# violetdenim/c3dgs

Measured on AMD Instinct MI355X. Metric: raster views/sec fwd+bwd @1920x1080, higher is better.
Workload: dtype f32; 1 GPU; BASELINE.json configs[2]: synth-v1 3M Gaussians, SH deg 3, indexed-camera rasterizer (QAT inner loop), mark_visible+fwd+bwd, 1 view/step/GPU; gaussians=3000000, width=1920, height=1080, sh_codebook=304096, gaussian_codebook=754096, parallelism=replicas x1

## Files before the change

### c3dgs_amd/csrc/backward_preprocess.hip

```cpp
#include "common.hpp"
#include "gsmath.hpp"

#ifndef C3DGS_BWD_CH
#define C3DGS_BWD_CH 128
#endif
#ifndef C3DGS_BWD_LONG_RUN
#define C3DGS_BWD_LONG_RUN 32
#endif
#ifndef C3DGS_BWD_FG
#define C3DGS_BWD_FG 8
#endif
#ifndef C3DGS_BWD_WAVES
#define C3DGS_BWD_WAVES 3
#endif

namespace c3dgs {

constexpr int SUM_WAVES = BWD_LIST / 64;
static_assert(BWD_LIST % 256 == 0 && BWD_LIST <= 1024, "a list is one workgroup of sum_partials_kernel and whole ones of backward_preprocess_kernel");

struct BwdArgs {
    int P, D, M, W, H;
    const float* means3D; const float* sh; const float* scales; const float* scale_factors; const float* rotations;
    const float* cov3D_precomp; const int64_t* sh_indices; const int64_t* g_indices;
    const float* view; const float* proj; const float* campos;
    float tan_fovx, tan_fovy, focal_x, focal_y, scale_modifier;
    const int32_t* radii; const uint32_t* inst_offset; const uint32_t* block_base; const uint8_t* clamped; const float4* splat;
    float* partials; const uint8_t* touched;
    uint32_t* live_count; uint32_t* live_ids; uint32_t* live_slots;
    c3dgs_raster_grads g;
};

template <int DEG>
__device__ __forceinline__ void sh_backward(const float* c, const f3 d0, const float g[3], float dmean_add[3], float* basis_out)
{
    const float len = sqrtf(d0.x * d0.x + d0.y * d0.y + d0.z * d0.z);
    const float x = d0.x / len, y = d0.y / len, z = d0.z / len;
    float dx[3] = { 0, 0, 0 }, dy[3] = { 0, 0, 0 }, dz[3] = { 0, 0, 0 };
    constexpr int NB = (DEG + 1) * (DEG + 1);
    float basis[NB];
    basis[0] = SH_C0;
    if (DEG > 0) {
        basis[1] = -SH_C1 * y; basis[2] = SH_C1 * z; basis[3] = -SH_C1 * x;
#pragma unroll
        for (int ch = 0; ch < 3; ch++) {
            dx[ch] = -SH_C1 * c[3 * 3 + ch];
            dy[ch] = -SH_C1 * c[1 * 3 + ch];
            dz[ch] = SH_C1 * c[2 * 3 + ch];
        }
    }
    if (DEG > 1) {
        const float xx = x * x, yy = y * y, zz = z * z, xy = x * y, yz = y * z, xz = x * z;
        basis[4] = SH_C2_0 * xy; basis[5] = SH_C2_1 * yz; basis[6] = SH_C2_2 * (2.f * zz - xx - yy);
        basis[7] = SH_C2_3 * xz; basis[8] = SH_C2_4 * (xx - yy);
#pragma unroll
        for (int ch = 0; ch < 3; ch++) {
            const float s4 = c[4 * 3 + ch], s5 = c[5 * 3 + ch], s6 = c[6 * 3 + ch], s7 = c[7 * 3 + ch], s8 = c[8 * 3 + ch];
            dx[ch] += SH_C2_0 * y * s4 + SH_C2_2 * 2.f * -x * s6 + SH_C2_3 * z * s7 + SH_C2_4 * 2.f * x * s8;
            dy[ch] += SH_C2_0 * x * s4 + SH_C2_1 * z * s5 + SH_C2_2 * 2.f * -y * s6 + SH_C2_4 * 2.f * -y * s8;
            dz[ch] += SH_C2_1 * y * s5 + SH_C2_2 * 2.f * 2.f * z * s6 + SH_C2_3 * x * s7;
        }
        if (DEG > 2) {
            basis[9] = SH_C3_0 * y * (3.f * xx - yy);
            basis[10] = SH_C3_1 * xy * z;
            basis[11] = SH_C3_2 * y * (4.f * zz - xx - yy);
            basis[12] = SH_C3_3 * z * (2.f * zz - 3.f * xx - 3.f * yy);
            basis[13] = SH_C3_4 * x * (4.f * zz - xx - yy);
            basis[14] = SH_C3_5 * z * (xx - yy);
            basis[15] = SH_C3_6 * x * (xx - 3.f * yy);
#pragma unroll
            for (int ch = 0; ch < 3; ch++) {
                const float s9 = c[9 * 3 + ch], s10 = c[10 * 3 + ch], s11 = c[11 * 3 + ch], s12 = c[12 * 3 + ch],
                            s13 = c[13 * 3 + ch], s14 = c[14 * 3 + ch], s15 = c[15 * 3 + ch];
                dx[ch] += SH_C3_0 * s9 * 3.f * 2.f * xy + SH_C3_1 * s10 * yz + SH_C3_2 * s11 * -2.f * xy +
                          SH_C3_3 * s12 * -3.f * 2.f * xz + SH_C3_4 * s13 * (-3.f * xx + 4.f * zz - yy) +
                          SH_C3_5 * s14 * 2.f * xz + SH_C3_6 * s15 * 3.f * (xx - yy);
                dy[ch] += SH_C3_0 * s9 * 3.f * (xx - yy) + SH_C3_1 * s10 * xz + SH_C3_2 * s11 * (-3.f * yy + 4.f * zz - xx) +
                          SH_C3_3 * s12 * -3.f * 2.f * yz + SH_C3_4 * s13 * -2.f * xy + SH_C3_5 * s14 * -2.f * yz +
                          SH_C3_6 * s15 * -3.f * 2.f * xy;
                dz[ch] += SH_C3_1 * s10 * xy + SH_C3_2 * s11 * 4.f * 2.f * yz + SH_C3_3 * s12 * 3.f * (2.f * zz - xx - yy) +
                          SH_C3_4 * s13 * 4.f * 2.f * xz + SH_C3_5 * s14 * (xx - yy);
            }
        }
    }
#pragma unroll
    for (int k = 0; k < NB; k++) basis_out[k] = basis[k];
    const float ddx = dx[0] * g[0] + dx[1] * g[1] + dx[2] * g[2];
    const float ddy = dy[0] * g[0] + dy[1] * g[1] + dy[2] * g[2];
    const float ddz = dz[0] * g[0] + dz[1] * g[1] + dz[2] * g[2];
    const float sum2 = d0.x * d0.x + d0.y * d0.y + d0.z * d0.z;
    const float invsum32 = 1.0f / sqrtf(sum2 * sum2 * sum2);
    dmean_add[0] = ((+sum2 - d0.x * d0.x) * ddx - d0.y * d0.x * ddy - d0.z * d0.x * ddz) * invsum32;
    dmean_add[1] = (-d0.x * d0.y * ddx + (sum2 - d0.y * d0.y) * ddy - d0.z * d0.y * ddz) * invsum32;
    dmean_add[2] = (-d0.x * d0.z * ddx - d0.y * d0.z * ddy + (sum2 - d0.z * d0.z) * ddz) * invsum32;
}

__device__ __forceinline__ uint32_t nth_set_bit(unsigned long long m, uint32_t r)
{
    uint32_t w = (uint32_t)m, at = 0, c = (uint32_t)__popc(w);
    if (r >= c) { r -= c; w = (uint32_t)(m >> 32); at = 32; }
    c = (uint32_t)__popc(w & 0xFFFFu); if (r >= c) { r -= c; w >>= 16; at += 16; }
    c = (uint32_t)__popc(w & 0xFFu);   if (r >= c) { r -= c; w >>= 8; at += 8; }
    c = (uint32_t)__popc(w & 0xFu);    if (r >= c) { r -= c; w >>= 4; at += 4; }
    c = (uint32_t)__popc(w & 0x3u);    if (r >= c) { r -= c; w >>= 2; at += 2; }
    if (r >= (w & 1u)) at += 1;
    return at;
}

__global__ void __launch_bounds__(BWD_LIST) __attribute__((amdgpu_waves_per_eu(8, 8))) sum_partials_kernel(const BwdArgs a)
{
    constexpr int SW = SUM_WAVES, LIST = BWD_LIST;
    const int i = blockIdx.x * LIST + threadIdx.x;
    const size_t si = (size_t)i;
    const c3dgs_raster_grads& o = a.g;

    constexpr int CH = C3DGS_BWD_CH;
    __shared__ float s_buf[SUM_WAVES][CH * PARTIAL_FLOATS];
#define s_stage(w, sl, q) s_buf[w][(sl) * PARTIAL_FLOATS + (q)]
    constexpr int FG = C3DGS_BWD_FG;
    __shared__ unsigned long long s_fl[SUM_WAVES][FG];
    __shared__ uint32_t s_pre[SUM_WAVES][FG + 1];
    bool any_written = false;
    float acc[PARTIAL_FLOATS];
#pragma unroll
    for (int q = 0; q < PARTIAL_FLOATS; q++) acc[q] = 0.f;
    const int lane_ = threadIdx.x & 63, wv = threadIdx.x >> 6;
    const unsigned long long lt_mask = (1ull << lane_) - 1ull;
    uint32_t start_;
    {
        const int ic = min(i, a.P - 1);
        const uint32_t end_ = a.inst_offset[ic] + a.block_base[ic >> 8];
        start_ = (ic == 0) ? 0u : a.inst_offset[ic - 1] + a.block_base[(ic - 1) >> 8];
        if (i >= a.P) start_ = end_;
        const uint32_t w_begin = __builtin_amdgcn_readfirstlane(start_);
        const uint32_t w_end = __builtin_amdgcn_readlane(end_, 63);
        for (uint32_t base = w_begin; base < w_end; base += FG * 64) {
            const uint32_t nsl = min((uint32_t)(FG * 64), w_end - base);
            uint32_t fbits = 0;
            uint8_t fb[FG];
#pragma unroll
            for (int g = 0; g < FG; g++) fb[g] = a.touched[base + min((uint32_t)(g * 64 + lane_), nsl - 1u)];
#pragma unroll
            for (int g = 0; g < FG; g++)
                if ((uint32_t)(g * 64 + lane_) < nsl && fb[g] != 0) fbits |= 1u << g;
            uint32_t W = 0;
            uint32_t pre[FG + 1];
#pragma unroll
            for (int g = 0; g < FG; g++) {
                const unsigned long long bm = __ballot((fbits >> g) & 1u);
                if (lane_ == 0) { s_fl[wv][g] = bm; s_pre[wv][g] = W; }
                pre[g] = W;
                W += (uint32_t)__popcll(bm);
            }
            pre[FG] = W;
            if (W == 0) continue;
            if (lane_ == 0) s_pre[wv][FG] = W;
            __builtin_amdgcn_fence(__ATOMIC_RELEASE, "wavefront");
            __builtin_amdgcn_wave_barrier();
            __builtin_amdgcn_fence(__ATOMIC_ACQUIRE, "wavefront");
            auto below = [&](uint32_t x) -> uint32_t {
                const uint32_t g = x >> 6;
                if (g >= (uint32_t)FG) return s_pre[wv][FG];
                return s_pre[wv][g] + (uint32_t)__popcll(s_fl[wv][g] & ((1ull << (x & 63u)) - 1ull));
            };
            const uint32_t lo = min(max(start_, base), base + nsl) - base, hi = min(max(end_, base), base + nsl) - base;
            const uint32_t clo = below(lo), chi = below(hi);
            any_written |= chi > clo;
            for (uint32_t p0 = 0; p0 < W; p0 += CH) {
                float st[CH / 64][PARTIAL_FLOATS];
#pragma unroll
                for (int h = 0; h < CH / 64; h++) {
                    const uint32_t e = min(p0 + (uint32_t)(h * 64 + lane_), W - 1u);
                    uint32_t g = 0, r = e;
#pragma unroll
                    for (int k = 1; k < FG; k++)
                        if (e >= pre[k]) { g = (uint32_t)k; r = e - pre[k]; }
                    const uint32_t slot = g * 64u + nth_set_bit(s_fl[wv][g], r);
                    const float* src = a.partials + (size_t)(base + slot) * PARTIAL_FLOATS;
#pragma unroll
                    for (int q = 0; q < PARTIAL_FLOATS; q++) st[h][q] = src[q];
                }
#pragma unroll
                for (int h = 0; h < CH / 64; h++)
#pragma unroll
                    for (int q = 0; q < PARTIAL_FLOATS; q++) s_stage(wv, h * 64 + lane_, q) = st[h][q];
                __builtin_amdgcn_fence(__ATOMIC_RELEASE, "wavefront");
                __builtin_amdgcn_wave_barrier();
                __builtin_amdgcn_fence(__ATOMIC_ACQUIRE, "wavefront");
                const uint32_t c_lo = max(clo, p0), c_hi = min(chi, p0 + CH);
                const bool long_run = c_hi > c_lo + (uint32_t)C3DGS_BWD_LONG_RUN;
                unsigned long long longm = __ballot(long_run);
                while (longm) {
                    const int owner = __ffsll((long long)longm) - 1;
                    longm &= longm - 1ull;
                    const uint32_t o_lo = (uint32_t)__shfl((int)c_lo, owner) - p0, o_hi = (uint32_t)__shfl((int)c_hi, owner) - p0;
                    float part[PARTIAL_FLOATS];
#pragma unroll
                    for (int q = 0; q < PARTIAL_FLOATS; q++) part[q] = 0.f;
                    for (uint32_t e = o_lo + (uint32_t)lane_; e < o_hi; e += 64u) {
#pragma unroll
                        for (int q = 0; q < PARTIAL_FLOATS; q++) part[q] += s_stage(wv, e, q);
                    }
#pragma unroll
                    for (int q = 0; q < PARTIAL_FLOATS; q++) {
#pragma unroll
                        for (int o = 32; o > 0; o >>= 1) part[q] += __shfl_xor(part[q], o);
                        if (lane_ == owner) acc[q] += part[q];
                    }
                }
                if (!long_run) {
                    for (uint32_t c = c_lo; c < c_hi; c++) {
#pragma unroll
                        for (int q = 0; q < PARTIAL_FLOATS; q++) acc[q] += s_stage(wv, c - p0, q);
                    }
                }
                __builtin_amdgcn_fence(__ATOMIC_RELEASE, "wavefront");
                __builtin_amdgcn_wave_barrier();
            }
        }
    }
    const bool live = any_written;
    const unsigned long long lm = __ballot(live);
    const bool per_gaussian_rows = !a.sh_indices && !a.g_indices;
    bool sh_rows_done = false;
    if (per_gaussian_rows && o.dL_dsh && a.sh && ((a.M * 3) & 3) == 0 && (reinterpret_cast<uintptr_t>(o.dL_dsh) & 15u) == 0) {
        sh_rows_done = true;
        const int r4 = (a.M * 3) >> 2;
        const int first = blockIdx.x * LIST + wv * 64;
        const int rows = min(64, a.P - first);
        float4* span = reinterpret_cast<float4*>(o.dL_dsh + (size_t)first * a.M * 3);
        int row = lane_ / r4, col = lane_ - row * r4;
        const int drow = 64 / r4, dcol = 64 - drow * r4;
        for (int q = lane_; q < rows * r4; q += 64) {
            if (!((lm >> row) & 1ull)) span[q] = make_float4(0.f, 0.f, 0.f, 0.f);
            row += drow; col += dcol;
            if (col >= r4) { col -= r4; row++; }
        }
    }
    if (i < a.P && !live) {
        if (o.dL_dmeans2D) { o.dL_dmeans2D[3 * si] = 0.f; o.dL_dmeans2D[3 * si + 1] = 0.f; o.dL_dmeans2D[3 * si + 2] = 0.f; }
        if (o.dL_dcolors) { o.dL_dcolors[3 * si] = 0.f; o.dL_dcolors[3 * si + 1] = 0.f; o.dL_dcolors[3 * si + 2] = 0.f; }
        if (o.dL_dopacity) o.dL_dopacity[si] = 0.f;
        if (o.dL_dmeans3D) { o.dL_dmeans3D[3 * si] = 0.f; o.dL_dmeans3D[3 * si + 1] = 0.f; o.dL_dmeans3D[3 * si + 2] = 0.f; }
        if (o.dL_dcov3D) for (int q = 0; q < 6; q++) o.dL_dcov3D[6 * si + q] = 0.f;
        if (o.dL_dscale_factors) o.dL_dscale_factors[si] = 0.f;
        if (per_gaussian_rows) {
            if (o.dL_dsh && a.sh && !sh_rows_done) for (int q = 0; q < a.M * 3; q++) o.dL_dsh[si * a.M * 3 + q] = 0.f;
            if (o.dL_dscales && a.scales) for (int q = 0; q < 3; q++) o.dL_dscales[3 * si + q] = 0.f;
            if (o.dL_drotations && a.scales) for (int q = 0; q < 4; q++) o.dL_drotations[4 * si + q] = 0.f;
        }
    }
    __shared__ uint32_t s_cnt[SW];
    if (lane_ == 0) s_cnt[wv] = (uint32_t)__popcll(lm);
    __syncthreads();
    uint32_t run0 = 0, all = 0;
#pragma unroll
    for (int w = 0; w < SW; w++) { const uint32_t c = s_cnt[w]; run0 += (w < wv) ? c : 0u; all += c; }
    if (live) {
        const size_t pos = (size_t)blockIdx.x * LIST + run0 + (uint32_t)__popcll(lm & lt_mask);
        a.live_ids[pos] = (uint32_t)i;
        a.live_slots[pos] = start_;
        float* dst = a.partials + (size_t)start_ * PARTIAL_FLOATS;
#pragma unroll
        for (int q = 0; q < PARTIAL_FLOATS; q++) dst[q] = acc[q];
    }
    if (threadIdx.x == 0) a.live_count[blockIdx.x] = all;
}
#undef s_stage

template <int DEG, bool INDEXED>
__global__ void __launch_bounds__(256)
#if C3DGS_BWD_WAVES
__attribute__((amdgpu_waves_per_eu(C3DGS_BWD_WAVES, C3DGS_BWD_WAVES)))
#endif
backward_preprocess_kernel(const BwdArgs a, const float* __restrict__ cam_view, const float* __restrict__ cam_proj,
                           const float* __restrict__ cam_pos)
{
    const uint32_t n_lists = gridDim.x / (BWD_LIST / 256);
    const uint32_t list = blockIdx.x % n_lists, quarter = blockIdx.x / n_lists;
    const uint32_t n_live = a.live_count[list];
    const uint32_t off = quarter * 256u + threadIdx.x;
    if ((off & ~63u) >= n_live) return;
    const size_t pos = (size_t)list * BWD_LIST + off;
    const bool live = off < n_live;
    const int i = live ? (int)a.live_ids[pos] : 0;
    const size_t si = (size_t)i;
    const c3dgs_raster_grads& o = a.g;
    constexpr int NB = (DEG + 1) * (DEG + 1);

    __shared__ float s_g[256][3];
    __shared__ int32_t s_row[256];
    __shared__ float s_ds[INDEXED ? 256 : 1][3];
    __shared__ float s_dq[INDEXED ? 256 : 1][4];
    __shared__ int32_t s_gi[INDEXED ? 256 : 1];
    __shared__ float s_bas[256][NB + 1];
#define s_basis(t, k) s_bas[t][k]
    s_row[threadIdx.x] = -1;
    if (INDEXED) s_gi[threadIdx.x] = -1;

    if (live) {
    float acc[PARTIAL_FLOATS];
    {
        const float* src = a.partials + (size_t)a.live_slots[pos] * PARTIAL_FLOATS;
#pragma unroll
        for (int q = 0; q < PARTIAL_FLOATS; q++) acc[q] = src[q];
    }
    const float4 rec0 = a.splat[3 * si], rec1 = a.splat[3 * si + 1];
    const f3 m = { a.means3D[3 * si], a.means3D[3 * si + 1], a.means3D[3 * si + 2] };
    const uint8_t cl = a.clamped[i];
    size_t gi = si, row = si;
    float sf = 1.f;
    if (INDEXED) {
        if (a.g_indices) gi = (size_t)a.g_indices[i];
        if (a.scale_factors) sf = a.scale_factors[i];
        if (a.sh_indices) row = (size_t)a.sh_indices[i];
    }
    float sc[3] = { 0, 0, 0 };
    float4 rot = make_float4(1, 0, 0, 0);
    float cov3D[6];
    if (a.cov3D_precomp) {
#pragma unroll
        for (int q = 0; q < 6; q++) cov3D[q] = a.cov3D_precomp[6 * si + q];
    } else {
        sc[0] = a.scales[3 * gi]; sc[1] = a.scales[3 * gi + 1]; sc[2] = a.scales[3 * gi + 2];
        rot = *reinterpret_cast<const float4*>(a.rotations + 4 * gi);
    }
    constexpr int NC = (DEG + 1) * (DEG + 1) * 3;
    float c[NC];
    if (a.sh) {
        const float* shp = a.sh + row * (size_t)a.M * 3;
        if ((a.M * 3) % 4 == 0 && NC % 4 == 0) {
#pragma unroll
            for (int q = 0; q < NC / 4; q++) {
                const float4 v = reinterpret_cast<const float4*>(shp)[q];
                c[4 * q] = v.x; c[4 * q + 1] = v.y; c[4 * q + 2] = v.z; c[4 * q + 3] = v.w;
            }
        } else {
#pragma unroll
            for (int q = 0; q < NC; q++) c[q] = shp[q];
        }
    }

    float sh_add[3] = { 0.f, 0.f, 0.f };
    if (a.sh) {
        const float g[3] = { (cl & 1) ? 0.f : acc[0], (cl & 2) ? 0.f : acc[1], (cl & 4) ? 0.f : acc[2] };
        const f3 d0 = { m.x - cam_pos[0], m.y - cam_pos[1], m.z - cam_pos[2] };
        float basis[NB];
        sh_backward<DEG>(c, d0, g, sh_add, basis);
        if (o.dL_dsh) {
#pragma unroll
            for (int k = 0; k < NB; k++) s_basis(threadIdx.x, k) = basis[k];
            s_g[threadIdx.x][0] = g[0]; s_g[threadIdx.x][1] = g[1]; s_g[threadIdx.x][2] = g[2];
            s_row[threadIdx.x] = (int32_t)row;
        }
    }

    const float k_a = rec0.z, k_b = rec0.w, k_c = rec1.x, opac = rec1.y;
    const float dcol[3] = { acc[0], acc[1], acc[2] };
    const float d2x = -0.5f * (float)a.W * opac * (k_a * acc[4] + k_b * acc[5]);
    const float d2y = -0.5f * (float)a.H * opac * (k_c * acc[5] + k_b * acc[4]);
    const float dcon_x = -0.5f * opac * acc[6], dcon_y = -0.5f * opac * acc[7], dcon_w = -0.5f * opac * acc[8];
    acc[8] = acc[3];
    if (o.dL_dcolors) { o.dL_dcolors[3 * si] = dcol[0]; o.dL_dcolors[3 * si + 1] = dcol[1]; o.dL_dcolors[3 * si + 2] = dcol[2]; }
    if (o.dL_dmeans2D) { o.dL_dmeans2D[3 * si] = d2x; o.dL_dmeans2D[3 * si + 1] = d2y; o.dL_dmeans2D[3 * si + 2] = 0.f; }
    if (o.dL_dopacity) o.dL_dopacity[si] = acc[8];

    if (!a.cov3D_precomp)
        cov3d_from_scale_rot(sc[0], sc[1], sc[2], INDEXED ? sf * a.scale_modifier : a.scale_modifier, rot, cov3D);
    const Cov2D cv = cov2d(m, a.focal_x, a.focal_y, a.tan_fovx, a.tan_fovy, cov3D, cam_view);
    const float limx = 1.3f * a.tan_fovx, limy = 1.3f * a.tan_fovy;
    const float x_grad_mul = (cv.txtz < -limx || cv.txtz > limx) ? 0.f : 1.f;
    const float y_grad_mul = (cv.tytz < -limy || cv.tytz > limy) ? 0.f : 1.f;
    const float A[2][3] = { { cv.T.c[0][0], cv.T.c[0][1], cv.T.c[0][2] }, { cv.T.c[1][0], cv.T.c[1][1], cv.T.c[1][2] } };
    const float Sg[3][3] = { { cov3D[0], cov3D[1], cov3D[2] }, { cov3D[1], cov3D[3], cov3D[4] }, { cov3D[2], cov3D[4], cov3D[5] } };
    const float ca = cv.a, cb = cv.b, cc = cv.c;
    const float denom = ca * cc - cb * cb;
    float dL_da = 0, dL_db = 0, dL_dc = 0;
    const float denom2inv = 1.0f / ((denom * denom) + 0.0000001f);
    float dcov[6] = { 0, 0, 0, 0, 0, 0 };
    if (denom2inv != 0) {
        dL_da = denom2inv * (-cc * cc * dcon_x + 2 * cb * cc * dcon_y + (denom - ca * cc) * dcon_w);
        dL_dc = denom2inv * (-ca * ca * dcon_w + 2 * ca * cb * dcon_y + (denom - ca * cc) * dcon_x);
        dL_db = denom2inv * 2 * (cb * cc * dcon_x - (denom + 2 * cb * cb) * dcon_y + ca * cb * dcon_w);
        const float Gm[2][2] = { { dL_da, 0.5f * dL_db }, { 0.5f * dL_db, dL_dc } };
        float S3[3][3];
#pragma unroll
        for (int u = 0; u < 3; u++)
#pragma unroll
            for (int v = u; v < 3; v++) {
                float s = 0.f;
#pragma unroll
                for (int q = 0; q < 2; q++)
#pragma unroll
                    for (int w = 0; w < 2; w++) s += A[q][u] * Gm[q][w] * A[w][v];
                S3[u][v] = s;
            }
        dcov[0] = S3[0][0]; dcov[3] = S3[1][1]; dcov[5] = S3[2][2];
        dcov[1] = 2.f * S3[0][1]; dcov[2] = 2.f * S3[0][2]; dcov[4] = 2.f * S3[1][2];
    }
    if (o.dL_dcov3D)
#pragma unroll
        for (int q = 0; q < 6; q++) o.dL_dcov3D[6 * si + q] = dcov[q];

    float AS[2][3], dA[2][3];
#pragma unroll
    for (int q = 0; q < 2; q++)
#pragma unroll
        for (int v = 0; v < 3; v++) AS[q][v] = A[q][0] * Sg[0][v] + A[q][1] * Sg[1][v] + A[q][2] * Sg[2][v];
#pragma unroll
    for (int v = 0; v < 3; v++) {
        dA[0][v] = 2 * AS[0][v] * dL_da + AS[1][v] * dL_db;
        dA[1][v] = 2 * AS[1][v] * dL_dc + AS[0][v] * dL_db;
    }
    const float* view = cam_view;
    const float dJ00 = view[0] * dA[0][0] + view[4] * dA[0][1] + view[8] * dA[0][2];
    const float dJ02 = view[2] * dA[0][0] + view[6] * dA[0][1] + view[10] * dA[0][2];
    const float dJ11 = view[1] * dA[1][0] + view[5] * dA[1][1] + view[9] * dA[1][2];
    const float dJ12 = view[2] * dA[1][0] + view[6] * dA[1][1] + view[10] * dA[1][2];
    const float tz = 1.f / cv.t.z, tz2 = tz * tz, tz3 = tz2 * tz;
    const float dtx = x_grad_mul * -a.focal_x * tz2 * dJ02;
    const float dty = y_grad_mul * -a.focal_y * tz2 * dJ12;
    const float dtz = -a.focal_x * tz2 * dJ00 - a.focal_y * tz2 * dJ11 + (2 * a.focal_x * cv.t.x) * tz3 * dJ02 +
                      (2 * a.focal_y * cv.t.y) * tz3 * dJ12;
    float dmean[3] = { view[0] * dtx + view[1] * dty + view[2] * dtz,
                       view[4] * dtx + view[5] * dty + view[6] * dtz,
                       view[8] * dtx + view[9] * dty + view[10] * dtz };

    const float* proj = cam_proj;
    const float4 mh = xform4x4(m, proj);
    const float m_w = 1.0f / (mh.w + 0.0000001f);
    const float mul1 = (proj[0] * m.x + proj[4] * m.y + proj[8] * m.z + proj[12]) * m_w * m_w;
    const float mul2 = (proj[1] * m.x + proj[5] * m.y + proj[9] * m.z + proj[13]) * m_w * m_w;
    dmean[0] += (proj[0] * m_w - proj[3] * mul1) * d2x + (proj[1] * m_w - proj[3] * mul2) * d2y;
    dmean[1] += (proj[4] * m_w - proj[7] * mul1) * d2x + (proj[5] * m_w - proj[7] * mul2) * d2y;
    dmean[2] += (proj[8] * m_w - proj[11] * mul1) * d2x + (proj[9] * m_w - proj[11] * mul2) * d2y;

    dmean[0] += sh_add[0]; dmean[1] += sh_add[1]; dmean[2] += sh_add[2];
    if (o.dL_dmeans3D) { o.dL_dmeans3D[3 * si] = dmean[0]; o.dL_dmeans3D[3 * si + 1] = dmean[1]; o.dL_dmeans3D[3 * si + 2] = dmean[2]; }

    if (a.scales) {
        const float s[3] = { (INDEXED ? sf * a.scale_modifier : a.scale_modifier) * sc[0],
                             (INDEXED ? sf * a.scale_modifier : a.scale_modifier) * sc[1],
                             (INDEXED ? sf * a.scale_modifier : a.scale_modifier) * sc[2] };
        const float r = rot.x, x = rot.y, y = rot.z, z = rot.w;
        const float Rm[3][3] = { { 1.f - 2.f * (y * y + z * z), 2.f * (x * y - r * z), 2.f * (x * z + r * y) },
                                 { 2.f * (x * y + r * z), 1.f - 2.f * (x * x + z * z), 2.f * (y * z - r * x) },
                                 { 2.f * (x * z - r * y), 2.f * (y * z + r * x), 1.f - 2.f * (x * x + y * y) } };
        const float G3[3][3] = { { dcov[0], 0.5f * dcov[1], 0.5f * dcov[2] },
                                 { 0.5f * dcov[1], dcov[3], 0.5f * dcov[4] },
                                 { 0.5f * dcov[2], 0.5f * dcov[4], dcov[5] } };
        float Q[3][3], d_s[3];
#pragma unroll
        for (int j = 0; j < 3; j++) {
            float col[3];
#pragma unroll
            for (int k = 0; k < 3; k++) {
                float accv = 0.f;
#pragma unroll
                for (int q = 0; q < 3; q++) accv += G3[k][q] * (Rm[q][j] * s[j]);
                col[k] = 2.0f * accv;
            }
            d_s[j] = Rm[0][j] * col[0] + Rm[1][j] * col[1] + Rm[2][j] * col[2];
#pragma unroll
            for (int k = 0; k < 3; k++) Q[k][j] = col[k] * s[j];
        }
        float dq[4];
        dq[0] = 2 * z * (Q[1][0] - Q[0][1]) + 2 * y * (Q[0][2] - Q[2][0]) + 2 * x * (Q[2][1] - Q[1][2]);
        dq[1] = 2 * y * (Q[0][1] + Q[1][0]) + 2 * z * (Q[0][2] + Q[2][0]) + 2 * r * (Q[2][1] - Q[1][2]) - 4 * x * (Q[2][2] + Q[1][1]);
        dq[2] = 2 * x * (Q[0][1] + Q[1][0]) + 2 * r * (Q[0][2] - Q[2][0]) + 2 * z * (Q[2][1] + Q[1][2]) - 4 * y * (Q[2][2] + Q[0][0]);
        dq[3] = 2 * r * (Q[1][0] - Q[0][1]) + 2 * x * (Q[0][2] + Q[2][0]) + 2 * y * (Q[2][1] + Q[1][2]) - 4 * z * (Q[1][1] + Q[0][0]);
        if (INDEXED) {
            s_ds[threadIdx.x][0] = d_s[0] * sf; s_ds[threadIdx.x][1] = d_s[1] * sf; s_ds[threadIdx.x][2] = d_s[2] * sf;
            s_dq[threadIdx.x][0] = dq[0]; s_dq[threadIdx.x][1] = dq[1]; s_dq[threadIdx.x][2] = dq[2]; s_dq[threadIdx.x][3] = dq[3];
            s_gi[threadIdx.x] = (int32_t)gi;
            if (o.dL_dscale_factors) o.dL_dscale_factors[si] = d_s[0] * sc[0] + d_s[1] * sc[1] + d_s[2] * sc[2];
        } else {
            if (o.dL_dscales) { o.dL_dscales[3 * si] = d_s[0]; o.dL_dscales[3 * si + 1] = d_s[1]; o.dL_dscales[3 * si + 2] = d_s[2]; }
            if (o.dL_drotations) *reinterpret_cast<float4*>(o.dL_drotations + 4 * si) = make_float4(dq[0], dq[1], dq[2], dq[3]);
        }
    } else if (INDEXED && o.dL_dscale_factors) {
        o.dL_dscale_factors[si] = 0.f;
    }
    }

    {
        __builtin_amdgcn_fence(__ATOMIC_RELEASE, "wavefront");
        __builtin_amdgcn_wave_barrier();
        __builtin_amdgcn_fence(__ATOMIC_ACQUIRE, "wavefront");
        const int lane = threadIdx.x & 63, wbase = threadIdx.x & ~63;
        if (o.dL_dsh && a.sh) {
            const int k = min(lane / 3, NB - 1), ch = lane - 3 * (lane / 3);
            for (int j = 0; j < 64; j++) {
                const int32_t row = s_row[wbase + j];
                if (row < 0) continue;
                float* dst = o.dL_dsh + (size_t)row * a.M * 3 + lane;
                const float v = s_basis(wbase + j, k) * s_g[wbase + j][ch];
                if (INDEXED) { if (lane < NB * 3) atomicAdd(dst, v); }
                else if (lane < a.M * 3) *dst = lane < NB * 3 ? v : 0.f;
            }
        }
    }
    if (INDEXED) {
        const int lane = threadIdx.x & 63, wbase = threadIdx.x & ~63;
        if (a.scales) {
            if (o.dL_dscales)
#pragma unroll
                for (int it = 0; it < 3; it++) {
                    const int q = it * 64 + lane, j = q / 3, c = q - 3 * j;
                    const int32_t gi = s_gi[wbase + j];
                    if (gi >= 0) atomicAdd(o.dL_dscales + 3 * (size_t)gi + c, s_ds[wbase + j][c]);
                }
            if (o.dL_drotations)
#pragma unroll
                for (int it = 0; it < 4; it++) {
                    const int q = it * 64 + lane, j = q >> 2, c = q & 3;
                    const int32_t gi = s_gi[wbase + j];
                    if (gi >= 0) atomicAdd(o.dL_drotations + 4 * (size_t)gi + c, s_dq[wbase + j][c]);
                }
        }
    }
}

void launch_backward_preprocess(const c3dgs_raster_params& p, const int32_t* radii, const GeomPtrs& g, const BwdPtrs& w,
                                const c3dgs_raster_grads& gr, hipStream_t s)
{
    if (p.P <= 0) return;
    BwdArgs a;
    a.P = p.P; a.D = p.D; a.M = p.M; a.W = p.W; a.H = p.H;
    a.means3D = p.means3D; a.sh = p.sh; a.scales = p.scales; a.scale_factors = p.scale_factors; a.rotations = p.rotations;
    a.cov3D_precomp = p.cov3D_precomp; a.sh_indices = p.sh_indices; a.g_indices = p.g_indices;
    a.view = p.viewmatrix; a.proj = p.projmatrix; a.campos = p.campos;
    a.tan_fovx = p.tan_fovx; a.tan_fovy = p.tan_fovy;
    a.focal_y = p.H / (2.0f * p.tan_fovy);
    a.focal_x = p.W / (2.0f * p.tan_fovx);
    a.scale_modifier = p.scale_modifier;
    a.radii = radii; a.inst_offset = g.inst_offset; a.block_base = g.block_base; a.clamped = g.clamped; a.splat = g.splat;
    a.partials = w.partials; a.touched = w.touched; a.g = gr;
    a.live_count = w.live_count; a.live_ids = w.live_ids; a.live_slots = w.live_slots;
    const int n_lists = (p.P + BWD_LIST - 1) / BWD_LIST;
    sum_partials_kernel<<<n_lists, BWD_LIST, 0, s>>>(a);
    const dim3 grid(n_lists * (BWD_LIST / 256)), block(256);
    const bool indexed = p.sh_indices != nullptr || p.g_indices != nullptr;
    const int deg = p.sh ? p.D : 0;
#define C3DGS_LAUNCH(DEG)                                                                     \
    do {                                                                                      \
        if (indexed) backward_preprocess_kernel<DEG, true><<<grid, block, 0, s>>>(a, a.view, a.proj, a.campos);         \
        else backward_preprocess_kernel<DEG, false><<<grid, block, 0, s>>>(a, a.view, a.proj, a.campos);                \
    } while (0)
    switch (deg) {
        case 0: C3DGS_LAUNCH(0); break;
        case 1: C3DGS_LAUNCH(1); break;
        case 2: C3DGS_LAUNCH(2); break;
        default: C3DGS_LAUNCH(3); break;
    }
#undef C3DGS_LAUNCH
}

#undef s_basis

}
```

### c3dgs_amd/csrc/common.hpp

```cpp
#pragma once
#include <hip/hip_runtime.h>
#include <cstdint>
#include <cstddef>
#include <cstdio>
#include <cstring>
#include <string>

#include "../../include/c3dgs_hip.h"

namespace c3dgs {

constexpr int TILE = 16;
constexpr int TILE_PIX = 256;
constexpr int SPLAT_F4 = 3;
constexpr int PARTIAL_FLOATS = 9;
constexpr int BWD_LIST = 1024;

void set_error(const std::string& msg);
inline int fail(int code, const std::string& msg) { set_error(msg); return code; }

#define C3DGS_HIP_TRY(expr)                                                                         \
    do {                                                                                            \
        hipError_t e__ = (expr);                                                                    \
        if (e__ != hipSuccess)                                                                      \
            return ::c3dgs::fail(C3DGS_E_HIP, std::string(#expr) + ": " + hipGetErrorString(e__));  \
    } while (0)

#define C3DGS_STAGE(name, debug, stream)                                                            \
    do {                                                                                            \
        hipError_t e__ = hipGetLastError();                                                         \
        if (e__ == hipSuccess && (debug)) e__ = hipStreamSynchronize(stream);                       \
        if (e__ != hipSuccess)                                                                      \
            return ::c3dgs::fail(C3DGS_E_HIP, std::string("stage ") + name + ": " + hipGetErrorString(e__)); \
    } while (0)

__device__ __forceinline__ uint32_t f2ord(float f)
{
    const uint32_t u = __float_as_uint(f);
    return (u & 0x80000000u) ? ~u : (u | 0x80000000u);
}
__device__ __host__ __forceinline__ float ord2f(uint32_t o)
{
    const uint32_t u = (o & 0x80000000u) ? (o & 0x7fffffffu) : ~o;
    float f;
    memcpy(&f, &u, 4);
    return f;
}

inline size_t align_up(size_t v, size_t a = 256) { return (v + a - 1) / a * a; }

size_t scan_temp_bytes(int P);
size_t sort_temp_bytes(int R, int end_bit, int key_bytes = 2);

inline int tiles_x(int W) { return (W + TILE - 1) / TILE; }
inline int tiles_y(int H) { return (H + TILE - 1) / TILE; }

inline uint32_t higher_msb(uint32_t n)
{
    uint32_t msb = sizeof(n) * 4, step = msb;
    while (step > 1) {
        step /= 2;
        if (n >> msb) msb += step; else msb -= step;
    }
    if (n >> msb) msb++;
    return msb;
}

inline void geom_layout(int P, c3dgs_geom_layout* L)
{
    size_t o = 0, p = (size_t)(P > 0 ? P : 1);
    L->splat = o;             o = align_up(o + p * SPLAT_F4 * 16);
    L->depth_keys = o;        o = align_up(o + p * 4);
    L->depth_keys_sorted = o; o = align_up(o + p * 4);
    L->depth_order = o;       o = align_up(o + p * 4);
    L->sorted_offsets = o;    o = align_up(o + p * 8);
    L->inst_offset = o;       o = align_up(o + p * 4);
    L->rects = o;             o = align_up(o + p * 8);
    L->clamped = o;           o = align_up(o + p);
    L->block_base = o;        o = align_up(o + ((p + 255) / 256 + 2) * 4);
    L->depth_base = o;        o = align_up(o + ((p + 255) / 256 + 1) * 4);
    L->scan_temp = o;         L->scan_temp_bytes = scan_temp_bytes((int)p);
    o = align_up(o + L->scan_temp_bytes);
    L->total_bytes = o;
}

inline size_t geom_gtab_bytes(const c3dgs_raster_params& p) { return (p.g_indices && p.scales) ? align_up((size_t)(p.GS > 0 ? p.GS : 1) * 32) : 0; }

inline int tile_key_bytes_for(long long T) { return T > 65536 ? 4 : 2; }
inline int tile_key_bytes(int W, int H) { return tile_key_bytes_for((long long)tiles_x(W) * tiles_y(H)); }
inline int tile_sort_end_bit_for(long long T)
{
    const int msb = (int)higher_msb((uint32_t)T), kbits = 8 * tile_key_bytes_for(T);
    return msb < kbits ? msb : kbits;
}
inline int tile_sort_end_bit(int W, int H) { return tile_sort_end_bit_for((long long)tiles_x(W) * tiles_y(H)); }

inline void binning_layout(int R, int W, int H, c3dgs_binning_layout* L)
{
    size_t o = 0, r = (size_t)(R > 0 ? R : 1);
    const int end_bit = tile_sort_end_bit(W, H);
    const size_t kb = (size_t)tile_key_bytes(W, H);
    L->keys_unsorted = o;   o = align_up(o + r * kb);
    L->values_unsorted = o; o = align_up(o + r * 4);
    L->keys_sorted = o;     o = align_up(o + r * kb);
    L->point_list = o;      o = align_up(o + r * 4);
    L->sort_temp = o;       L->sort_temp_bytes = sort_temp_bytes((int)r, end_bit, (int)kb);
    o = align_up(o + L->sort_temp_bytes);
    L->total_bytes = o;
}

struct ImageLayout : c3dgs_image_layout { size_t tile_used_c, n_contrib_c; };
inline void image_layout(int W, int H, ImageLayout* L)
{
    size_t o = 0, n = (size_t)W * H, t = (size_t)tiles_x(W) * tiles_y(H);
    L->final_T = o;     o = align_up(o + n * 4);
    L->n_contrib = o;   o = align_up(o + n * 4);
    L->ranges = o;      o = align_up(o + t * 8);
    L->tile_used = o;   o = align_up(o + t * 4);
    L->tile_order = o;  o = align_up(o + t * 4);
    L->tile_used_c = o; o = align_up(o + t * 4);
    L->n_contrib_c = o; o = align_up(o + n * 4);
    L->total_bytes = o;
}

struct CompactBinLayout { size_t cqm, cid, bin_bytes; };
inline CompactBinLayout compact_bin_layout(int R)
{
    const size_t r = (size_t)(R > 0 ? R : 1);
    CompactBinLayout C;
    C.cqm = 0; C.cid = align_up(r); C.bin_bytes = C.cid + align_up(r * 4);
    return C;
}

inline void backward_layout(int P, int R, c3dgs_backward_layout* L)
{
    size_t o = 0, r = (size_t)(R > 0 ? R : 1), n_lists = ((size_t)(P > 0 ? P : 1) + BWD_LIST - 1) / BWD_LIST;
    L->partials = o;   o = align_up(o + r * PARTIAL_FLOATS * sizeof(float));
    L->touched = o;    o = align_up(o + r);
    L->live_ids = o;   o = align_up(o + n_lists * BWD_LIST * 4);
    L->live_slots = o; o = align_up(o + n_lists * BWD_LIST * 4);
    L->live_count = o; o = align_up(o + n_lists * 4);
    L->list_len = BWD_LIST;
    L->total_bytes = o;
}

struct DepthBackwardLayout { size_t dz, total_bytes; };
inline DepthBackwardLayout depth_backward_layout(int P, int R)
{
    c3dgs_backward_layout B; backward_layout(P, R, &B);
    const size_t r = (size_t)(R > 0 ? R : 1);
    DepthBackwardLayout L;
    L.dz = B.total_bytes;
    L.total_bytes = align_up(L.dz + r * sizeof(float));
    return L;
}

struct ContribSlot { float sum, max; uint32_t hits; };
struct ContribLayout { size_t slots, touched, touched_bytes, total_bytes; };
inline ContribLayout contrib_layout(int P, int R)
{
    (void)P;
    size_t o = 0, r = (size_t)(R > 0 ? R : 1);
    ContribLayout L;
    L.slots = o;   o = align_up(o + r * sizeof(ContribSlot));
    L.touched = o; o = align_up(o + r);
    L.touched_bytes = o - L.touched;
    L.total_bytes = o;
    return L;
}

struct ErrorLayout { size_t slots, touched, touched_bytes, total_bytes; };
inline ErrorLayout error_layout(int P, int R)
{
    (void)P;
    size_t o = 0, r = (size_t)(R > 0 ? R : 1);
    ErrorLayout L;
    L.slots = o;   o = align_up(o + r * sizeof(float));
    L.touched = o; o = align_up(o + r);
    L.touched_bytes = o - L.touched;
    L.total_bytes = o;
    return L;
}

constexpr int SPARSE_ADAM_SELECT_ROWS = 256;
struct SparseAdamLayout { size_t count, rows, block_base, total_bytes; };
inline SparseAdamLayout sparse_adam_layout(int64_t P)
{
    const size_t p = (size_t)(P > 0 ? P : 1);
    SparseAdamLayout L;
    size_t o = 0;
    L.count = o;      o = align_up(o + 4);
    L.rows = o;       o = align_up(o + p * 4);
    L.block_base = o; o = align_up(o + ((p + SPARSE_ADAM_SELECT_ROWS - 1) / SPARSE_ADAM_SELECT_ROWS + 2) * 4);
    L.total_bytes = o;
    return L;
}

struct GeomPtrs {
    float4* splat; uint32_t* depth_keys; uint32_t* depth_keys_sorted;
    uint32_t* depth_order; uint2* sorted_offsets; uint32_t* inst_offset; uint16_t* rects;
    uint8_t* clamped; uint32_t* block_base; uint32_t* depth_base; void* scan_temp; size_t scan_temp_bytes;
    float4* gtab;
};
struct BinPtrs {
    void* keys_unsorted; uint32_t* values_unsorted; void* keys_sorted; uint32_t* point_list;
    void* sort_temp; size_t sort_temp_bytes; int key_bytes;
};
struct ImgPtrs { float* final_T; uint32_t* n_contrib; uint2* ranges; uint32_t* tile_used; uint32_t* tile_order;
                 uint32_t* tile_used_c; uint32_t* n_contrib_c; };
struct CompactPtrs { uint8_t* cqm; uint32_t* cid; };
struct BwdPtrs { float* partials; uint8_t* touched; size_t touched_bytes;
                 uint32_t* live_ids; uint32_t* live_slots; uint32_t* live_count; };
struct ContribPtrs { ContribSlot* slots; uint8_t* touched; size_t touched_bytes; };
struct ErrorPtrs { float* slots; uint8_t* touched; size_t touched_bytes; };

inline GeomPtrs geom_ptrs(void* base, int P)
{
    c3dgs_geom_layout L; geom_layout(P, &L);
    char* b = (char*)base;
    return { (float4*)(b + L.splat), (uint32_t*)(b + L.depth_keys), (uint32_t*)(b + L.depth_keys_sorted), (uint32_t*)(b + L.depth_order),
             (uint2*)(b + L.sorted_offsets), (uint32_t*)(b + L.inst_offset), (uint16_t*)(b + L.rects),
             (uint8_t*)(b + L.clamped), (uint32_t*)(b + L.block_base), (uint32_t*)(b + L.depth_base), (void*)(b + L.scan_temp),
             L.scan_temp_bytes, (float4*)(b + L.total_bytes) };
}
inline BinPtrs bin_ptrs(void* base, int R, int W, int H)
{
    c3dgs_binning_layout L; binning_layout(R, W, H, &L);
    char* b = (char*)base;
    return { (void*)(b + L.keys_unsorted), (uint32_t*)(b + L.values_unsorted), (void*)(b + L.keys_sorted),
             (uint32_t*)(b + L.point_list), (void*)(b + L.sort_temp), L.sort_temp_bytes, tile_key_bytes(W, H) };
}
inline ImgPtrs img_ptrs(void* base, int W, int H)
{
    ImageLayout L; image_layout(W, H, &L);
    char* b = (char*)base;
    return { (float*)(b + L.final_T), (uint32_t*)(b + L.n_contrib), (uint2*)(b + L.ranges), (uint32_t*)(b + L.tile_used),
             (uint32_t*)(b + L.tile_order), (uint32_t*)(b + L.tile_used_c), (uint32_t*)(b + L.n_contrib_c) };
}
inline CompactPtrs compact_ptrs(const BinPtrs& bp, int R)
{
    const CompactBinLayout C = compact_bin_layout(R);
    return { (uint8_t*)bp.sort_temp + C.cqm, (uint32_t*)((char*)bp.sort_temp + C.cid) };
}
inline BwdPtrs bwd_ptrs(void* base, int P, int R)
{
    c3dgs_backward_layout L; backward_layout(P, R, &L);
    char* b = (char*)base;
    return { (float*)(b + L.partials), (uint8_t*)(b + L.touched), L.live_ids - L.touched,
             (uint32_t*)(b + L.live_ids), (uint32_t*)(b + L.live_slots), (uint32_t*)(b + L.live_count) };
}

inline ContribPtrs contrib_ptrs(void* base, int P, int R)
{
    const ContribLayout L = contrib_layout(P, R);
    char* b = (char*)base;
    return { (ContribSlot*)(b + L.slots), (uint8_t*)(b + L.touched), L.touched_bytes };
}

inline ErrorPtrs error_ptrs(void* base, int P, int R)
{
    const ErrorLayout L = error_layout(P, R);
    char* b = (char*)base;
    return { (float*)(b + L.slots), (uint8_t*)(b + L.touched), L.touched_bytes };
}

void launch_camera_from_pose(const float* pose, float inv_tan_x, float inv_tan_y, float* view, float* proj, float* campos, hipStream_t s);
void launch_mark_visible(int P, const float* means3D, const float* view, uint8_t* present, hipStream_t s);
void launch_mark_visible_pose(int P, const float* means3D, const float* pose7, uint8_t* present, hipStream_t s);
void launch_pack_codebook(const c3dgs_raster_params& p, float4* gtab, hipStream_t s);
void launch_preprocess(const c3dgs_raster_params& p, const GeomPtrs& g, int32_t* radii, uint2* ranges, void* zero_span, size_t zero_n16,
                       hipStream_t s);
void launch_scan_blocks(int nb, uint32_t* base, const uint32_t* sort_err, uint32_t* host_out, uint32_t host_seq, hipStream_t s);
void launch_depth_order_scan(int P, const GeomPtrs& g, hipStream_t s);
void launch_duplicate_with_keys(int P, const GeomPtrs& g, const BinPtrs& b, int grid_x, const uint32_t* sort_err,
                                void* zero_span, size_t zero_n16, hipStream_t s);
void launch_identify_ranges(int R, const void* keys_sorted, int key_bytes, uint2* ranges, const uint32_t* sort_err, hipStream_t s);
hipError_t run_depth_sort(void* temp, size_t temp_bytes, const uint32_t* kin, uint32_t* kout, const uint32_t* vin,
                          uint32_t* vout, int P, const uint2* rects, uint2* rects_sorted, hipStream_t s, bool ctrl_cleared = false,
                          bool rects_fit_bytes = false, bool hist_done = false);
hipError_t run_depth_hist_scan(void* temp, size_t temp_bytes, const uint32_t* keys, int P, int nb, uint32_t* base,
                               const uint32_t* sort_err, uint32_t* host_out, uint32_t host_seq, hipStream_t s);
hipError_t run_tile_sort(void* temp, size_t temp_bytes, const void* kin, void* kout, int key_bytes, const uint32_t* vin,
                         uint32_t* vout, int R, int end_bit, hipStream_t s, bool ctrl_cleared = false);
size_t depth_sort_clear_bytes(int P);
size_t tile_sort_clear_bytes(int R, int end_bit, int key_bytes);
bool onesweep_enabled();
int onesweep_timed_out(hipStream_t s);
uint32_t* onesweep_error_word();
size_t onesweep_depth_temp_bytes(int P);
size_t onesweep_tile_temp_bytes(int R, int end_bit, int key_bytes = 2);
size_t onesweep_depth_clear_bytes(int P);
size_t onesweep_tile_clear_bytes(int R, int end_bit, int key_bytes);
hipError_t onesweep_depth_sort(void* temp, size_t temp_bytes, const uint32_t* kin, uint32_t* kout, const uint32_t* vin, uint32_t* vout,
                               int P, const uint2* gather_src, uint2* gather_dst, hipStream_t s, bool ctrl_cleared = false,
                               bool rects_fit_bytes = false, bool hist_done = false);
hipError_t onesweep_depth_hist_scan(void* temp, size_t temp_bytes, const uint32_t* keys, int P, int nb, uint32_t* base,
                                    const uint32_t* sort_err, uint32_t* host_out, uint32_t host_seq, hipStream_t s);
hipError_t onesweep_tile_sort32(void* temp, size_t temp_bytes, const uint32_t* kin, uint32_t* kout, const uint32_t* vin, uint32_t* vout,
                                int R, int end_bit, hipStream_t s, bool ctrl_cleared = false);
hipError_t onesweep_tile_sort(void* temp, size_t temp_bytes, const uint16_t* kin, uint16_t* kout, const uint32_t* vin, uint32_t* vout,
                              int R, int end_bit, hipStream_t s, bool ctrl_cleared = false);
void launch_render_forward(int W, int H, const ImgPtrs& img, const uint32_t* point_list, const float4* splat,
                           const float* bg, float* out_color, const CompactPtrs& cl, const uint32_t* sort_err, hipStream_t s);
void launch_backward_prep(int W, int H, const ImgPtrs& img, void* zero_a, size_t n16_a, void* zero_b, size_t n16_b, hipStream_t s);
void launch_render_backward(int W, int H, const ImgPtrs& img, const float4* splat,
                            const uint32_t* block_base, const float* bg, const float* dL_dpix, float* partials,
                            uint8_t* touched, const CompactPtrs& cl, void* zero_span, size_t zero_n16, hipStream_t s);
void launch_render_depth(int W, int H, const ImgPtrs& img, const CompactPtrs& cl, const float4* splat, const uint32_t* depth_keys,
                         float* out_depth, float* out_alpha, float* out_median, const uint32_t* sort_err, hipStream_t s);
void launch_render_depth_backward(int W, int H, const ImgPtrs& img, const CompactPtrs& cl, const GeomPtrs& g, const BwdPtrs& w,
                                  float* dz_plane, const float* dL_ddepth, const float* dL_dalpha, const uint32_t* sort_err,
                                  hipStream_t s);
void launch_depth_backward_fold(int P, const GeomPtrs& g, const BwdPtrs& w, const float* dz_plane, const float* view,
                                float* dL_dmeans3D, const uint32_t* sort_err, hipStream_t s);
void launch_render_contrib(int W, int H, const ImgPtrs& img, const CompactPtrs& cl, const GeomPtrs& g, const ContribPtrs& w,
                           const uint32_t* sort_err, hipStream_t s);
void launch_contrib_sum(int P, const GeomPtrs& g, const ContribPtrs& w, float* out_sum, float* out_max, uint32_t* out_hits,
                        const uint32_t* sort_err, hipStream_t s);
void launch_contrib_accumulate(int P_model, int P_rows, const uint8_t* visible, const int32_t* rank, const float* weight_sum,
                               const float* weight_max, const uint32_t* hits, float* acc_sum, float* acc_max, int64_t* acc_hits,
                               uint32_t* acc_views, hipStream_t s);
void launch_render_error(int W, int H, const ImgPtrs& img, const CompactPtrs& cl, const GeomPtrs& g, const ErrorPtrs& w,
                         const float* pixel_map, const uint32_t* sort_err, hipStream_t s);
void launch_error_sum(int P, const GeomPtrs& g, const ErrorPtrs& w, float* out_sum, const uint32_t* sort_err, hipStream_t s);
void launch_error_accumulate(int P_model, int P_rows, const uint8_t* visible, const int32_t* rank, const float* err_sum,
                             float* acc_max, float* acc_sum, hipStream_t s);
void launch_error_map_l1(int C, int H, int W, const float* img, const float* gt, float* out, hipStream_t s);
struct PoseGradIn {
    int P, D, M; float scale_modifier;
    const float* means3D; const float* dL_dmeans3D; const float* dL_dcov3D; const float* dL_dcolors;
    const float* sh; const int64_t* sh_indices;
    const float* cov3D_precomp; const float* scales; const float* rotations; const float* scale_factors; const int64_t* g_indices;
    const uint8_t* clamped; const int32_t* radii; const float* pose;
};
size_t pose_grad_workspace_bytes(int P);
void launch_pose_sums(const PoseGradIn& in, float* rows, hipStream_t s);
void launch_pose_fold(int P, const float* rows, const float* pose, float* out, hipStream_t s);
void launch_backward_preprocess(const c3dgs_raster_params& p, const int32_t* radii, const GeomPtrs& g, const BwdPtrs& w,
                                const c3dgs_raster_grads& gr, hipStream_t s);
int launch_weighted_distance(int64_t N, int C, int K, const float* coefs, const int64_t* gather, const float* codebook,
                             float* out_dist, int64_t* out_idx, hipStream_t s, void* ws = nullptr, size_t ws_bytes = 0, int presplit = -1);
bool wd_presplit_supported(int C, int K, const float* coefs, const float* codebook, const void* ws, size_t ws_bytes);
int launch_vq_apply_split(int K, int D, float* S, float* codebook, float* entry_importance, float decay, float alpha, float eps,
                          int scale_normalize, void* ws, size_t ws_bytes, int parity, hipStream_t s);
void launch_vq_seed_words(int K, int D, void* ws, hipStream_t s);
uint32_t* vq_next_absmax_word(int K, int D, void* ws, int parity);
size_t wd_ws_bytes(int64_t N, int C, int K);
int launch_wd_debug_scores(int64_t N, int C, int K, const float* coefs, const float* codebook, float* scores, void* ws, size_t ws_bytes,
                           float* out_dist, int64_t* out_idx, hipStream_t s);
void launch_vq_accumulate(int64_t B, int K, int D, const float* x, const float* w, const int64_t* gather,
                          const int64_t* idx, const float* dist, float* S, double* dist_sum, hipStream_t s, uint32_t* clear_word = nullptr);
void launch_vq_apply(int K, int D, const float* S, float* codebook, float* entry_importance, float decay, float alpha,
                     float eps, int scale_normalize, hipStream_t s);

size_t morton_workspace_bytes(int P);
int run_morton_order(int P, const float* xyz, int64_t* codes_out, int64_t* order_out, void* workspace, hipStream_t s);
void launch_extract_rot_scale(int n, const float* cov6, float* rot, float* scale, hipStream_t s);
size_t knn_workspace_bytes(int P);
int run_knn_sort(int P, const float* xyz, void* workspace, hipStream_t s);
void launch_knn_bounds(int P, void* workspace, hipStream_t s);
void launch_knn_query(int P, const void* workspace, float* out, hipStream_t s);
void launch_knn_query_neighbours(int P, const void* workspace, int32_t* idx, float* d2, hipStream_t s);
size_t ray_fill_plan_workspace_bytes(int P, long long rows);
hipError_t run_ray_fill_plan(int P, const float* d2, float step, long long capacity, int32_t* src, uint8_t* slot, int32_t* level,
                             int32_t* totals, void* workspace, size_t workspace_bytes, hipStream_t s, std::string* problem);
void launch_ray_fill_xyz(int P, const float* xyz, const int32_t* idx, const float* d2, float step, long long n_new,
                         const int32_t* src, const uint8_t* slot, const int32_t* level, float* out, hipStream_t s);
void launch_image_from_u8(int Hs, int Ws, int C, const uint8_t* src, int flip, const float* bg, int Hd, int Wd, float* out,
                          hipStream_t s);
void launch_adam(int n_tensors, const c3dgs_adam_tensor* tensors, double beta1, double beta2, double eps, hipStream_t s);
void launch_abs_accumulate(int64_t n, const float* g, float* acc, hipStream_t s);
void launch_sparse_adam_select(int64_t P, const void* mask, int mask_kind, void* workspace, hipStream_t s);
void launch_sparse_adam_step(int n_tensors, const c3dgs_sparse_adam_tensor* tensors, int64_t P, const void* workspace, double beta1,
                             double beta2, double eps, hipStream_t s);
void launch_densify_classify(int P, const float* accum, const float* denom, const float* scale_clone, const float* scale_split,
                             const float* scale_prune_self, const float* scale_prune_child, const float* opacity, float max_grad,
                             float dense_extent, float min_opacity, float big_extent, uint8_t* code, hipStream_t s);
size_t rows_plan_workspace_bytes(int P);
hipError_t run_rows_plan(int P, const uint8_t* code, int N, long long capacity, int32_t* src, uint8_t* kind, int32_t* draw_row,
                         int32_t* totals, void* workspace, hipStream_t s);
void launch_rows_apply(int P, long long P_new, const int32_t* src, const uint8_t* kind, const int32_t* draw_row, int n_tensors,
                       const c3dgs_rows_tensor* tensors, int N, long long n_draws, const float* rotation_raw, const float* std,
                       const float* z, int log_scaling, int half_xyz, hipStream_t s);
void launch_densify_stats(int P, const float* grad, const uint8_t* filter, const int32_t* radii, float* accum, float* denom,
                          float* max_radii, hipStream_t s);
size_t index_plan_workspace_bytes(int P, int K0, int K1);
hipError_t run_index_plan(int P, const uint8_t* keep, const int64_t* idx0, int K0, const int64_t* idx1, int K1, long long cap_rows,
                          long long cap_cb0, long long cap_cb1, int32_t* src, int64_t* new_idx0, int64_t* new_idx1, int32_t* cb_src0,
                          int32_t* cb_src1, int32_t* totals, void* workspace, hipStream_t s);
void launch_l1_ssim_value(const double* sums, double l1_scale, double ssim_scale, double constant, float* out, hipStream_t s);
void launch_l1_ssim_forward(int C, int H, int W, const float* img, const float* gt, float* Dmu, float* Ds1, float* Ds12,
                            double* sums, hipStream_t s);
void launch_l1_ssim_backward(int C, int H, int W, const float* img, const float* gt, const float* Dmu, const float* Ds1,
                             const float* Ds12, const float* grad_loss, float l1_coeff, float ssim_coeff, float* dL_dimg,
                             hipStream_t s);
constexpr int64_t IMAGE_METRICS_MAX_WORKGROUPS = (int64_t(1) << 24) - 1;
int64_t image_metrics_workgroups(int N, int C, int H, int W);
size_t image_metrics_ws_bytes(int N, int C, int H, int W);
void launch_image_metrics(int N, int C, int H, int W, const float* img, const float* gt, double* partials, double* out,
                          hipStream_t s);

size_t qat_workspace_bytes();
size_t qat_scan_bytes(int P);
void launch_qat_observe(const c3dgs_qat_params& q, void* workspace, hipStream_t s);
void launch_qat_codebooks(const c3dgs_qat_params& q, float* scales_n, float* rotations, float* shs, hipStream_t s);
void launch_qat_codebooks_backward(const c3dgs_qat_params& q, const float* g_scales, const float* g_rot, const float* g_shs,
                                   float* d_scaling, float* d_rotation, float* d_dc, float* d_rest, hipStream_t s);
hipError_t run_qat_visible(const c3dgs_qat_params& q, const float* view, uint8_t* visible, int32_t* rank, int32_t* count,
                           void* scan_ws, hipStream_t s);
void launch_qat_points(const c3dgs_qat_params& q, const uint8_t* visible, const int32_t* rank, const int64_t* sh_idx,
                       const int64_t* g_idx, float* means3D, float* opac, float* sfac, int64_t* sh_out, int64_t* g_out,
                       hipStream_t s);
void launch_qat_points_backward(const c3dgs_qat_params& q, const uint8_t* visible, const int32_t* rank, const float* g_m3,
                                const float* g_m2, const float* g_op, const float* g_sf, float* d_xyz, float* d_screen,
                                float* d_op, float* d_sf, hipStream_t s);
void launch_qat_quantize(const c3dgs_qat_params& q, int scaling_exp, int8_t* opacity, int8_t* scaling, int8_t* scaling_factor,
                         int8_t* rotation, int8_t* features_dc, int8_t* features_rest, hipStream_t s);
void launch_fake_quantize(long long n, const float* x, c3dgs_fq_state* state, int observe, int enabled, float c, float* out,
                          void* workspace, hipStream_t s);
void launch_fake_quantize_backward(long long n, const float* x, const c3dgs_fq_state* state, int enabled, const float* g,
                                   float* dx, hipStream_t s);

}
```

Measured before the change: 636.2 views/s.

## Store per-Gaussian partial sums in a coalesced wave-strided buffer for backward preprocess

The summed partial gradients for live Gaussians now go into a new dense live_sums buffer indexed by list position. Each wave of 64 gets a structure-of-arrays block, so stores and loads are coalesced. Before, they went to scattered per-instance slots that the consumer read through an indirect live_slots index. The consumer loads the three colour gradients first and defers the rest until after the SH work, to cut register pressure. Index arithmetic is narrowed to 32-bit, and the workspace grows by one extra partials-sized array per list.

```diff
diff --git a/c3dgs_amd/csrc/backward_preprocess.hip b/c3dgs_amd/csrc/backward_preprocess.hip
--- a/c3dgs_amd/csrc/backward_preprocess.hip
+++ b/c3dgs_amd/csrc/backward_preprocess.hip
@@ -27,7 +27,7 @@
     float tan_fovx, tan_fovy, focal_x, focal_y, scale_modifier;
     const int32_t* radii; const uint32_t* inst_offset; const uint32_t* block_base; const uint8_t* clamped; const float4* splat;
     float* partials; const uint8_t* touched;
-    uint32_t* live_count; uint32_t* live_ids; uint32_t* live_slots;
+    uint32_t* live_count; uint32_t* live_ids; float* live_sums;
     c3dgs_raster_grads g;
 };
 
@@ -259,10 +259,9 @@
     if (live) {
         const size_t pos = (size_t)blockIdx.x * LIST + run0 + (uint32_t)__popcll(lm & lt_mask);
         a.live_ids[pos] = (uint32_t)i;
-        a.live_slots[pos] = start_;
-        float* dst = a.partials + (size_t)start_ * PARTIAL_FLOATS;
-#pragma unroll
-        for (int q = 0; q < PARTIAL_FLOATS; q++) dst[q] = acc[q];
+        float* dst = a.live_sums + live_sums_index(pos);
+#pragma unroll
+        for (int q = 0; q < PARTIAL_FLOATS; q++) dst[q * 64] = acc[q];
     }
     if (threadIdx.x == 0) a.live_count[blockIdx.x] = all;
 }
@@ -300,20 +299,22 @@
 
     if (live) {
     float acc[PARTIAL_FLOATS];
+    const float* src;
     {
-        const float* src = a.partials + (size_t)a.live_slots[pos] * PARTIAL_FLOATS;
-#pragma unroll
-        for (int q = 0; q < PARTIAL_FLOATS; q++) acc[q] = src[q];
+        const uint32_t blk = (uint32_t)__builtin_amdgcn_readfirstlane((int)(list * (uint32_t)(BWD_LIST / 64) + (off >> 6)));
+        src = a.live_sums + (size_t)blk * (64 * PARTIAL_FLOATS) + (threadIdx.x & 63u);
+#pragma unroll
+        for (int q = 0; q < 3; q++) acc[q] = src[q * 64];
     }
     const float4 rec0 = a.splat[3 * si], rec1 = a.splat[3 * si + 1];
     const f3 m = { a.means3D[3 * si], a.means3D[3 * si + 1], a.means3D[3 * si + 2] };
     const uint8_t cl = a.clamped[i];
-    size_t gi = si, row = si;
+    uint32_t gi = (uint32_t)i, row = (uint32_t)i;
     float sf = 1.f;
     if (INDEXED) {
-        if (a.g_indices) gi = (size_t)a.g_indices[i];
+        if (a.g_indices) gi = (uint32_t)a.g_indices[i];
         if (a.scale_factors) sf = a.scale_factors[i];
-        if (a.sh_indices) row = (size_t)a.sh_indices[i];
+        if (a.sh_indices) row = (uint32_t)a.sh_indices[i];
     }
     float sc[3] = { 0, 0, 0 };
     float4 rot = make_float4(1, 0, 0, 0);
@@ -322,8 +323,8 @@
 #pragma unroll
         for (int q = 0; q < 6; q++) cov3D[q] = a.cov3D_precomp[6 * si + q];
     } else {
-        sc[0] = a.scales[3 * gi]; sc[1] = a.scales[3 * gi + 1]; sc[2] = a.scales[3 * gi + 2];
-        rot = *reinterpret_cast<const float4*>(a.rotations + 4 * gi);
+        sc[0] = a.scales[3 * (size_t)gi]; sc[1] = a.scales[3 * (size_t)gi + 1]; sc[2] = a.scales[3 * (size_t)gi + 2];
+        rot = *reinterpret_cast<const float4*>(a.rotations + 4 * (size_t)gi);
     }
     constexpr int NC = (DEG + 1) * (DEG + 1) * 3;
     float c[NC];
@@ -355,6 +356,8 @@
         }
     }
 
+#pragma unroll
+    for (int q = 3; q < PARTIAL_FLOATS; q++) acc[q] = src[q * 64];
     const float k_a = rec0.z, k_b = rec0.w, k_c = rec1.x, opac = rec1.y;
     const float dcol[3] = { acc[0], acc[1], acc[2] };
     const float d2x = -0.5f * (float)a.W * opac * (k_a * acc[4] + k_b * acc[5]);
@@ -536,7 +539,7 @@
     a.scale_modifier = p.scale_modifier;
     a.radii = radii; a.inst_offset = g.inst_offset; a.block_base = g.block_base; a.clamped = g.clamped; a.splat = g.splat;
     a.partials = w.partials; a.touched = w.touched; a.g = gr;
-    a.live_count = w.live_count; a.live_ids = w.live_ids; a.live_slots = w.live_slots;
+    a.live_count = w.live_count; a.live_ids = w.live_ids; a.live_sums = w.live_sums;
     const int n_lists = (p.P + BWD_LIST - 1) / BWD_LIST;
     sum_partials_kernel<<<n_lists, BWD_LIST, 0, s>>>(a);
     const dim3 grid(n_lists * (BWD_LIST / 256)), block(256);
diff --git a/c3dgs_amd/csrc/common.hpp b/c3dgs_amd/csrc/common.hpp
--- a/c3dgs_amd/csrc/common.hpp
+++ b/c3dgs_amd/csrc/common.hpp
@@ -132,7 +132,7 @@
     return C;
 }
 
-inline void backward_layout(int P, int R, c3dgs_backward_layout* L)
+inline void backward_layout(int P, int R, c3dgs_backward_layout* L, size_t* live_sums = nullptr)
 {
     size_t o = 0, r = (size_t)(R > 0 ? R : 1), n_lists = ((size_t)(P > 0 ? P : 1) + BWD_LIST - 1) / BWD_LIST;
     L->partials = o;   o = align_up(o + r * PARTIAL_FLOATS * sizeof(float));
@@ -140,9 +140,13 @@
     L->live_ids = o;   o = align_up(o + n_lists * BWD_LIST * 4);
     L->live_slots = o; o = align_up(o + n_lists * BWD_LIST * 4);
     L->live_count = o; o = align_up(o + n_lists * 4);
+    if (live_sums) *live_sums = o;
+    o = align_up(o + n_lists * BWD_LIST * PARTIAL_FLOATS * sizeof(float));
     L->list_len = BWD_LIST;
     L->total_bytes = o;
 }
+
+__host__ __device__ inline size_t live_sums_index(size_t pos) { return (pos >> 6) * (64 * PARTIAL_FLOATS) + (pos & 63); }
 
 struct DepthBackwardLayout { size_t dz, total_bytes; };
 inline DepthBackwardLayout depth_backward_layout(int P, int R)
@@ -210,7 +214,7 @@
                  uint32_t* tile_used_c; uint32_t* n_contrib_c; };
 struct CompactPtrs { uint8_t* cqm; uint32_t* cid; };
 struct BwdPtrs { float* partials; uint8_t* touched; size_t touched_bytes;
-                 uint32_t* live_ids; uint32_t* live_slots; uint32_t* live_count; };
+                 uint32_t* live_ids; uint32_t* live_slots; uint32_t* live_count; float* live_sums; };
 struct ContribPtrs { ContribSlot* slots; uint8_t* touched; size_t touched_bytes; };
 struct ErrorPtrs { float* slots; uint8_t* touched; size_t touched_bytes; };
 
@@ -244,10 +248,11 @@
 }
 inline BwdPtrs bwd_ptrs(void* base, int P, int R)
 {
-    c3dgs_backward_layout L; backward_layout(P, R, &L);
+    c3dgs_backward_layout L; size_t sums; backward_layout(P, R, &L, &sums);
     char* b = (char*)base;
     return { (float*)(b + L.partials), (uint8_t*)(b + L.touched), L.live_ids - L.touched,
-             (uint32_t*)(b + L.live_ids), (uint32_t*)(b + L.live_slots), (uint32_t*)(b + L.live_count) };
+             (uint32_t*)(b + L.live_ids), (uint32_t*)(b + L.live_slots), (uint32_t*)(b + L.live_count),
+             (float*)(b + sums) };
 }
 
 inline ContribPtrs contrib_ptrs(void* base, int P, int R)
```

After: 635.5 views/s. No clear change (-0.1%).
